# ParthaEth/GIF

Measured on AMD Instinct MI355X. Metric: G+D train-step images/sec at 256x256, batch 32/GPU, higher is better.
Workload: dtype f32

## Files before the change

### gif_amd/_lib.py

```python
import ctypes
import os

import torch

_HERE = os.path.dirname(os.path.abspath(__file__))
LIB_PATH = os.path.join(_HERE, "libgif_hip.so")

c_int, c_i64, c_float, c_void_p = ctypes.c_int, ctypes.c_int64, ctypes.c_float, ctypes.c_void_p


def knob(name, default):
    if os.environ.get("GIF_EXPERIMENTAL", "0") in ("", "0"):
        return default
    return os.environ.get(name, default)
P = c_void_p


class ConvGeom(ctypes.Structure):
    _fields_ = [(n, ctypes.c_int32) for n in ("B", "Hb", "Wb", "Cb", "Hs", "Ws", "Cs", "KH", "KW", "stride", "pad")]


class ConvEpilogue(ctypes.Structure):
    _fields_ = [("in_scale", P), ("out_scale", P), ("bias", P), ("residual", P),
                ("act", ctypes.c_int32), ("slope", c_float), ("gain", c_float),
                ("mask_src", P), ("mask_slope", c_float), ("mask_gain", c_float),
                ("dot_src", P), ("dot", P), ("colsum", P), ("red_ws", P), ("out_f32", ctypes.c_int32)]


class LinearBankSeg(ctypes.Structure):
    _fields_ = [("w", P), ("bias", P), ("s", P), ("gs", P), ("gw", P), ("gbias", P), ("n", ctypes.c_int32), ("reserved", ctypes.c_int32)]


GP, EP = ctypes.POINTER(ConvGeom), ctypes.POINTER(ConvEpilogue)

PROTOTYPES = {
    "gif_last_error": (ctypes.c_char_p, []),
    "gif_abi_version": (c_int, []),
    "gif_f16_overflow_clear": (c_int, [P]),
    "gif_f16_overflow_or_into": (c_int, [P, P]),
    "gif_f16_overflow_watch": (c_int, [c_int]),
    "gif_set_fp32_mfma_mode": (c_int, [c_int]),
    "gif_get_fp32_mfma_mode": (c_int, []),
    "gif_rasterize_workspace_bytes": (c_i64, [c_int, c_int, c_int, c_int]),
    "gif_rasterize_assume_clean_workspace": (c_int, [P, c_int]),
    "gif_rasterize_f32": (c_int, [P, P, P, P, c_int, c_int, c_int, c_int, P, P]),
    "gif_rasterize_colors_f32": (c_int, [P, P, P, P, P, c_int, c_int, c_int, c_int, P, P]),
    "gif_rasterize_f64": (c_int, [P, P, P, P, c_int, c_int, c_int, c_int, P, P]),
    "gif_rasterize_colors_f64": (c_int, [P, P, P, P, P, c_int, c_int, c_int, c_int, P, P]),
    "gif_rasterize_colors_bwd_workspace_bytes": (c_i64, [c_int, c_int, c_int, c_int]),
# ... 132 lines not shown
```

### gif_amd/csrc/common.h

```cpp
#pragma once
#include <hip/hip_runtime.h>
#include <stdint.h>
#include <stdio.h>
#include <stdlib.h>

#include "gif_hip.h"

#ifndef GIF_X3_FIRST_TERM
#define GIF_X3_FIRST_TERM 0
#endif

namespace gif {

void set_error(const char* fmt, ...);

inline int check_launch(const char* what) {
    hipError_t e = hipGetLastError();
    if (e != hipSuccess) {
        set_error("%s: %s", what, hipGetErrorString(e));
        return (int)e;
    }
    return 0;
}

#define GIF_REQUIRE(cond, ...)                \
    do {                                      \
        if (!(cond)) {                        \
            ::gif::set_error(__VA_ARGS__);    \
            return GIF_EINVAL;                \
        }                                     \
    } while (0)

inline hipStream_t as_stream(gif_stream_t s) { return reinterpret_cast<hipStream_t>(s); }

inline const char* knob(const char* name) {
    static const bool on = [] { const char* e = ::getenv("GIF_EXPERIMENTAL"); return e && atoi(e) != 0; }();
    return on ? ::getenv(name) : nullptr;
}

inline int cdiv(long a, long b) { return (int)((a + b - 1) / b); }

#if defined(__HIP_DEVICE_COMPILE__)
typedef __amdgpu_buffer_rsrc_t buf_rsrc_t;
__device__ __forceinline__ buf_rsrc_t make_buf_rsrc(const void* base, unsigned bytes) {
    return __builtin_amdgcn_make_buffer_rsrc(const_cast<void*>(base), 0, bytes, 0x00020000);
}
__device__ __forceinline__ void buf_load_lds16(buf_rsrc_t r, __attribute__((address_space(3))) void* lds, unsigned voff, int soff) {
    __builtin_amdgcn_raw_ptr_buffer_load_lds(r, lds, 16, (int)voff, soff, 0, 0);
}
#else
struct buf_rsrc_t {};
__device__ __forceinline__ buf_rsrc_t make_buf_rsrc(const void*, unsigned) { return {}; }
__device__ __forceinline__ void buf_load_lds16(buf_rsrc_t, __attribute__((address_space(3))) void*, unsigned, int) {}
#endif

constexpr int kMaxDevices = 64;
int current_device();
const float* zero_page16();
unsigned* f16_sat_flag();
struct LdsAttr {
    unsigned long granted[kMaxDevices] = {};
    void ensure(const void* kernel, size_t bytes);
};
// ... 114 lines not shown
```

### gif_amd/csrc/conv_igemm.hip

```cpp
#include <stdlib.h>

#include <atomic>
#include <type_traits>

#include "common.h"

#ifdef GIF_X3_TIMING_PROBE
__device__ unsigned long long g_x3_probe[12];
extern "C" int gif_debug_x3_probe_read(unsigned long long* out8, int reset) {
    hipDeviceSynchronize();
    if (hipMemcpyFromSymbol(out8, HIP_SYMBOL(g_x3_probe), 96) != hipSuccess) return -1;
    if (reset) {
        unsigned long long z[12] = {0, 0, 0, 0, 0, 0, 0, 0, 0, 0, 0, 0};
        if (hipMemcpyToSymbol(HIP_SYMBOL(g_x3_probe), z, 96) != hipSuccess) return -1;
    }
    return 0;
}
#endif

namespace {

typedef float f32x16 __attribute__((ext_vector_type(16)));
typedef float f32x4 __attribute__((ext_vector_type(4)));

// ... 7 lines not shown
    const float* bias;
    const void* residual;
    int B, Hi, Wi, Ci;
    int Ho, Wo, Co;
    int Hp, Wp;
    int os, ooy, oox;
    int is;
    int ntaps, nky, nkx, dy0, ddy, dx0, ddx, ky0, kx0, kstep, KW;
    int RP, CP;
    int act;
    float slope, gain;
    int M;
    int tiles_m, tiles_n;
    int stab_nb, stab_stride;
    const void* zero;
    int m_begin;
    int x3;
    const int* wexp;
    unsigned* gate;
    unsigned gate_gen;
    unsigned* h2_stats;
    const void* mask_src;
    const void* dot_src;
    float mask_slope, mask_gain;
    float* part_cs;
    float* part_dot;
    int part_row0;
    int part_cap;
    int no_split;
    unsigned* sat_flag;
    int out_f32;
    int pair;
    int dense;
    int t2_tx, t2_ty;
    int halo_dbg;
};

thread_local int t_part_rows = 0;
thread_local int t_last_bm = 0;

__device__ __forceinline__ int xcd_remap(int bid, int nwg) {
    const int nx = 8;
    int xcd = bid % nx, idx = bid / nx;
    int q = nwg / nx, r = nwg % nx;
    int base = xcd < r ? xcd * (q + 1) : r * (q + 1) + (xcd - r) * q;
    return base + idx;
// ... 6 lines not shown
    const T* const res = static_cast<const T*>(p.residual);
    T* const yout = static_cast<T*>(p.y);
    constexpr int LDC = BN + 4;
    constexpr int ROWTAB = 3;
    constexpr int STAGE_FLOATS = LDS_FLOATS ? LDS_FLOATS : 2 * (BM + BN) * LD;
    constexpr int EPI_CHUNKS = (BM * (LDC + ROWTAB) <= STAGE_FLOATS) ? 1 : (BM / 2 * (LDC + ROWTAB) <= STAGE_FLOATS) ? 2
                               : (BM / 4 * (LDC + ROWTAB) <= STAGE_FLOATS) ? 4 : 8;
    constexpr int CR = BM / EPI_CHUNKS;
    static_assert(CR % 32 == 0 && CR * (LDC + ROWTAB) <= STAGE_FLOATS && CR <= THREADS, "epilogue chunk must fit the staging LDS");
    float* Cs = smem;
    unsigned long long* const roff = reinterpret_cast<unsigned long long*>(Cs + CR * LDC);
    int* const rsmp = reinterpret_cast<int*>(roff + CR);
    constexpr unsigned long long NO_ROW = ~0ull;
    constexpr int C4_ROW = BN / 4;
    constexpr int EROWS = THREADS / C4_ROW;
    constexpr int E_IT = CR / EROWS;
    static_assert(CR % EROWS == 0, "epilogue row mapping");
    const int e_row0 = tid / C4_ROW, e_c = (tid % C4_ROW) * 4;
    const int n = n0 + e_c;
    float4 bias4 = make_float4(0.f, 0.f, 0.f, 0.f);
    if (p.bias && n < p.Co) bias4 = *reinterpret_cast<const float4*>(p.bias + n);
    const T* const msk = static_cast<const T*>(p.mask_src);
    const T* const dsrc = static_cast<const T*>(p.dot_src);
    const bool fused = msk || dsrc || p.part_cs || p.part_dot;
#if defined(GIF_EPI_PROBE) && GIF_EPI_PROBE == 3
    {
        float sacc = 0.f;
#pragma unroll
        for (int i = 0; i < MT; ++i)
#pragma unroll
            for (int j = 0; j < NT; ++j)
#pragma unroll
                for (int r = 0; r < 16; ++r) sacc += acc[i][j][r];
        if (m0 + wm0 < p.M) yout[(size_t)(m0 + wm0) * p.Co + n0 + wn0 + (tid & 63)] = (T)sacc;
        return;
    }
#endif
    float4 cs = make_float4(0.f, 0.f, 0.f, 0.f), ds = make_float4(0.f, 0.f, 0.f, 0.f);
    int osb = 0;
    f32x4 osc0 = {1.f, 1.f, 1.f, 1.f}, osc1 = osc0;
    constexpr bool OSC = sizeof(T) == 4;
    if (OSC && p.out_scale && n < p.Co) {
        osb = T2D ? t2_b : (m0 < p.M ? m0 : p.M - 1) / HWp;
        osc0 = *reinterpret_cast<const f32x4*>(p.out_scale + (size_t)osb * p.Co + n);
        osc1 = *reinterpret_cast<const f32x4*>(p.out_scale + (size_t)(osb + 1 < p.B ? osb + 1 : osb) * p.Co + n);
    }
// ... 71 lines not shown
                    for (int k = 0; k < PF; ++k) {
                        if (!ok[k]) continue;
                        float4 v = vv[k];
                        if constexpr (sizeof(T) != 4) v = *reinterpret_cast<const float4*>(Cs + (e_row0 + (it0 + k) * EROWS) * LDC + e_c);
                        if (FUSED && dsrc) {
                            ds.x += v.x * xa[k].x; ds.y += v.y * xa[k].y; ds.z += v.z * xa[k].z; ds.w += v.w * xa[k].w;
                        }
                        if (p.out_scale) {
                            f32x4 d = bs[k] == osb ? os0 : os1;
                            if (!OSC || __builtin_expect(bs[k] > osb + 1, 0)) d = *reinterpret_cast<const f32x4*>(p.out_scale + (size_t)bs[k] * p.Co + n);
                            const float dx = d[0], dy = d[1], dz = d[2], dw = d[3];
                            v.x *= dx; v.y *= dy; v.z *= dz; v.w *= dw;
                        }
                        if (res) {
                            float4 rv = gif::load4(res + off[k]);
                            v.x += rv.x; v.y += rv.y; v.z += rv.z; v.w += rv.w;
                        }
                        v.x += bias4.x; v.y += bias4.y; v.z += bias4.z; v.w += bias4.w;
                        if (p.act) {
                            v.x = (v.x > 0.f ? v.x : v.x * p.slope) * p.gain; v.y = (v.y > 0.f ? v.y : v.y * p.slope) * p.gain;
                            v.z = (v.z > 0.f ? v.z : v.z * p.slope) * p.gain; v.w = (v.w > 0.f ? v.w : v.w * p.slope) * p.gain;
                        }
                        if (FUSED) {
                            if (msk) {
                                const float4 xs = two_src ? xb[k] : xa[k];
                                v.x *= p.mask_gain * (xs.x > 0.f ? 1.f : p.mask_slope); v.y *= p.mask_gain * (xs.y > 0.f ? 1.f : p.mask_slope);
                                v.z *= p.mask_gain * (xs.z > 0.f ? 1.f : p.mask_slope); v.w *= p.mask_gain * (xs.w > 0.f ? 1.f : p.mask_slope);
                            }
                            cs.x += v.x; cs.y += v.y; cs.z += v.z; cs.w += v.w;
                        }
#ifdef GIF_NOSTORE_PROBE
                        if (p.M < 0)
#endif
                        {
                            if (sizeof(T) == 2 && p.out_f32) gif::store4(static_cast<float*>(p.y) + off[k], v);
                            else gif::store4_flag(yout + off[k], v, p.sat_flag);
                        }
                    }
                }
            };
            if (fused) rows(std::true_type{});
            else rows(std::false_type{});
        }
    }
    if (p.part_cs || p.part_dot) {
        __syncthreads();
// ... 1611 lines not shown
    GIF_REQUIRE(g->KH >= 1 && g->KH <= 3 && g->KW >= 1 && g->KW <= 3, "%s: kernel %dx%d unsupported", who, g->KH, g->KW);
    GIF_REQUIRE(g->stride == 1 || g->stride == 2, "%s: stride %d unsupported", who, g->stride);
    GIF_REQUIRE(g->pad >= 0, "%s: negative pad", who);
    GIF_REQUIRE((g->Hs - 1) * g->stride + g->KH - g->pad <= g->Hb + g->pad &&
                    (g->Ws - 1) * g->stride + g->KW - g->pad <= g->Wb + g->pad,
                "%s: small grid %dx%d does not fit big grid %dx%d (k=%d s=%d p=%d)", who, g->Hs, g->Ws, g->Hb,
                g->Wb, g->KH, g->stride, g->pad);
    return 0;
}

void fill_epilogue(GatherParams& p, const gif_conv_epilogue* e) {
    p.in_scale = e ? e->in_scale : nullptr;
    p.out_scale = e ? e->out_scale : nullptr;
    p.bias = e ? e->bias : nullptr;
    p.residual = e ? e->residual : nullptr;
    p.act = e ? e->act : 0;
    p.slope = e ? e->slope : 0.f;
    p.gain = e ? e->gain : 1.f;
    p.mask_src = e ? e->mask_src : nullptr;
    p.mask_slope = e ? e->mask_slope : 1.f;
    p.mask_gain = e ? e->mask_gain : 1.f;
    p.dot_src = e ? e->dot_src : nullptr;
    p.sat_flag = nullptr;
    p.out_f32 = e ? e->out_f32 : 0;
}

int check_tapdense(const gif_conv_geom* g, const gif_conv_epilogue* e, int cin, bool transposed, const char* who) {
    GIF_REQUIRE(gif_conv2d_x3_tapdense_steps(cin, g->KH, g->KW) > 0, "%s: tap-dense mode needs a 3x3 kernel and 8 <= Cin < 32 (got %dx%d, %d)",
                who, g->KH, g->KW, cin);
    GIF_REQUIRE(!transposed || g->stride == 1, "%s: tap-dense mode: a strided data gradient runs tap subsets per output phase", who);
    GIF_REQUIRE(!(e && e->in_scale), "%s: tap-dense mode has no per-sample input scales", who);
    return 0;
}

struct FusedSums {
    float* colsum = nullptr;
    float* dot = nullptr;
    float* part_cs = nullptr;
    float* part_dot = nullptr;
    float* tmp = nullptr;
    long cap = 0;

    bool active() const { return colsum || dot; }

    int begin(GatherParams& p, const gif_conv_epilogue* e, long out_rows, int Co, int B, long hw, bool single_phase, const char* who) {
        t_part_rows = 0;
        if (!e || (!e->colsum && !e->dot)) return 0;
// ... 48 lines not shown
        p.gate = gt.word; p.gate_gen = gt.gen;
        p.h2_stats = gif::h2_stats_words();
    }
    return 0;
}
inline void h2_to_fallback(GatherParams& p, const void* wp3) {
    p.x3 = 1;
    p.wp = wp3;
    p.wexp = nullptr;
}

template <typename T>
int check_channels(const gif_conv_geom* g, const char* who) {
    if (sizeof(T) == 2)
        GIF_REQUIRE(g->Cb % 8 == 0 && g->Cs % 8 == 0, "%s: f16 channel counts must be multiples of 8 (Cb=%d Cs=%d)", who, g->Cb, g->Cs);
    return 0;
}

template <typename T>
int conv2d_fwd_impl(const void* big, const void* wp, void* small, const gif_conv_geom* g, const gif_conv_epilogue* e,
                    gif_stream_t stream, const char* who, int x3 = 0, bool dense = false, const void* wp_fallback = nullptr) {
    if (int rc = check_geom(g, who)) return rc;
    if (int rc = check_channels<T>(g, who)) return rc;
    if (g->B == 0) return 0;
    GIF_REQUIRE(big && wp && small, "%s: null pointer", who);
    GatherParams p{};
    p.x = big; p.wp = wp; p.y = small; p.x3 = x3;
    fill_epilogue(p, e);
    if (sizeof(T) == 2) p.sat_flag = gif::f16_sat_flag();
    p.B = g->B; p.Hi = g->Hb; p.Wi = g->Wb; p.Ci = g->Cb;
    p.Ho = g->Hs; p.Wo = g->Ws; p.Co = g->Cs;
    p.Hp = g->Hs; p.Wp = g->Ws; p.os = 1; p.ooy = 0; p.oox = 0; p.is = g->stride;
    p.nky = g->KH; p.nkx = g->KW; p.ntaps = g->KH * g->KW;
    p.dy0 = -g->pad; p.ddy = 1; p.dx0 = -g->pad; p.ddx = 1;
    p.ky0 = 0; p.kx0 = 0; p.kstep = 1; p.KW = g->KW;
    pack_dims<T>(p.Co, p.Ci, &p.RP, &p.CP, x3 != 0);
    p.pair = (sizeof(T) == 2 && p.CP == 32) ? 1 : 0;
    if (dense) {
        if (int rc = check_tapdense(g, e, g->Cb, false, who)) return rc;
        p.dense = g->Cb / 4;
    }
    if (x3 == 2)
        if (int rc = h2_operands(p, wp, wp_fallback, gif::as_stream(stream))) return rc;
    p.M = p.B * p.Hp * p.Wp;
    double flops = 2.0 * p.M * (double)p.Co * p.Ci * p.ntaps;
    const int fam = sizeof(T) == 2 ? 6 : dense ? (x3 == 2 ? 17 : 12) : x3 == 2 ? 13 : x3 ? 8 : (p.Ci >= 32 ? 0 : 5);
// ... 1 lines not shown
    if (int rc = sums.begin(p, e, p.M, p.Co, p.B, (long)p.Hp * p.Wp, true, who)) return rc;
    gif::ProfScope prof(fam, flops, gif::as_stream(stream), p.M, p.Co, p.Ci, p.ntaps * 10 + g->stride);
    if (int rc = launch<T>(p, gif::as_stream(stream))) return rc;
    if (x3 == 2 && p.gate && wp_fallback) {
        const int rows2 = t_part_rows, bm2 = t_last_bm;
        h2_to_fallback(p, wp_fallback);
        t_part_rows = 0;
        if (int rc = launch<T>(p, gif::as_stream(stream))) return rc;
        if (sums.active() && (t_part_rows != rows2 || t_last_bm != bm2)) {
            gif::set_error("%s: the guarded bf16x3 twin tiles the op differently from the f16x2 launch (%d x %d vs %d x %d rows): fused "
                           "column sums would mix partials", who, t_part_rows, t_last_bm, rows2, bm2);
            return GIF_ENOSUP;
        }
    }
    if (int rc = sums.finish(p.Co, p.B, (long)p.Hp * p.Wp, gif::as_stream(stream), who)) return rc;
    return gif::check_launch(who);
}

template <typename T>
int conv2d_bwd_data_impl(const void* small, const void* wp, void* big, const gif_conv_geom* g, const gif_conv_epilogue* e,
                         gif_stream_t stream, const char* who, int x3 = 0, bool dense = false, const void* wp_fallback = nullptr) {
    if (int rc = check_geom(g, who)) return rc;
    if (int rc = check_channels<T>(g, who)) return rc;
    if (g->B == 0) return 0;
    GIF_REQUIRE(small && wp && big, "%s: null pointer", who);
    hipStream_t s = gif::as_stream(stream);
    GatherParams base{};
    base.x = small; base.wp = wp; base.y = big; base.x3 = x3;
    fill_epilogue(base, e);
    if (sizeof(T) == 2) base.sat_flag = gif::f16_sat_flag();
    base.B = g->B; base.Hi = g->Hs; base.Wi = g->Ws; base.Ci = g->Cs;
    base.Ho = g->Hb; base.Wo = g->Wb; base.Co = g->Cb;
    pack_dims<T>(base.Co, base.Ci, &base.RP, &base.CP, x3 != 0);
    base.pair = (sizeof(T) == 2 && base.CP == 32) ? 1 : 0;
    if (x3 == 2)
        if (int rc = h2_operands(base, wp, wp_fallback, s)) return rc;
    if (dense) {
        if (int rc = check_tapdense(g, e, g->Cs, true, who)) return rc;
        base.dense = g->Cs / 4;
    }
    const int st = g->stride;
    FusedSums sums;
    if (int rc = sums.begin(base, e, (long)g->B * g->Hb * g->Wb, base.Co, g->B, (long)g->Hb * g->Wb, st == 1, who)) return rc;
    auto pmod = [st](int a) { return ((a % st) + st) % st; };
    GatherParams ph[4];
    int nph = 0;
    bool need_zero = false;
    for (int py = 0; py < st; ++py)
        for (int px = 0; px < st; ++px) {
            GatherParams p = base;
            p.Hp = (g->Hb - py + st - 1) / st;
            p.Wp = (g->Wb - px + st - 1) / st;
            if (p.Hp <= 0 || p.Wp <= 0) continue;
            p.os = st; p.ooy = py; p.oox = px; p.is = 1;
            p.ky0 = pmod(py + g->pad); p.kx0 = pmod(px + g->pad); p.kstep = st; p.KW = g->KW;
            p.nky = p.ky0 < g->KH ? (g->KH - p.ky0 + st - 1) / st : 0;
            p.nkx = p.kx0 < g->KW ? (g->KW - p.kx0 + st - 1) / st : 0;
            p.ntaps = p.nky * p.nkx;
            p.dy0 = (py + g->pad - p.ky0) / st; p.ddy = -1;
            p.dx0 = (px + g->pad - p.kx0) / st; p.ddx = -1;
            if (p.ntaps == 0) { need_zero = true; continue; }
            p.M = p.B * p.Hp * p.Wp;
            ph[nph++] = p;
        }
    if (need_zero) {
        GIF_REQUIRE(!(e && (e->bias || e->residual || e->act || e->mask_src || e->colsum || e->dot)), "%s: epilogue unsupported with empty phases", who);
        hipError_t me = hipMemsetAsync(big, 0, (size_t)g->B * g->Hb * g->Wb * g->Cb * sizeof(T), s);
        if (me != hipSuccess) { gif::set_error("%s memset: %s", who, hipGetErrorString(me)); return (int)me; }
    }
    double flops = 2.0 * g->B * (double)g->Hs * g->Ws * g->KH * g->KW * (double)g->Cs * g->Cb;
    {
        const int fam = sizeof(T) == 2 ? 6 : dense ? (x3 == 2 ? 17 : 12) : x3 == 2 ? 13 : x3 ? 8 : (base.Ci >= 32 ? 0 : 5);
        gif::ProfScope prof(fam, flops, s, g->B * g->Hb * g->Wb, base.Co, base.Ci, -(g->KH * g->KW * 10 + g->stride));
        auto run_phases = [&]() -> int {
            bool merged = false;
            if (nph > 1 && conv_variant() == 0) {
                TileCfg c = pick_cfg<T>(base.Co, base.Ci);
                if (x3) c.BK = 32;
                bool small_all = c.BN == 128 && (sizeof(T) == 2 || c.BK == 32);
                for (int i = 0; i < nph && small_all; ++i)
                    small_all = (long)gif::cdiv(ph[i].M, 128) * (ph[i].RP / 128) < 384 &&
                                (long)ph[i].B * ph[i].Hi * ph[i].Wi * ph[i].Ci < (1L << 31) &&
                                (long)ph[i].B * ph[i].Ho * ph[i].Wo * ph[i].Co < (1L << 31);
                if (small_all)
                    merged = launch_multi<T>(ph, nph, base.in_scale != nullptr, s) == 0;
                if constexpr (sizeof(T) == 4) {
                    static const int big_multi_off = gif::knob("GIF_X3_MULTI_BIG") ? atoi(gif::knob("GIF_X3_MULTI_BIG")) == 0 : 0;
                    bool big_all = x3 && !small_all && !big_multi_off && c.BN == 128;
                    for (int i = 0; i < nph && big_all; ++i)
// ... 135 lines not shown
```

### gif_amd/csrc/conv_winograd.hip

```cpp
#include <stdlib.h>
#include <string.h>

#include "common.h"

namespace {

typedef float f32x16 __attribute__((ext_vector_type(16)));
typedef float f32x4 __attribute__((ext_vector_type(4)));

__device__ __forceinline__ int xcd_remap(int bid, int nwg) {
    const int nx = 8;
    int xcd = bid % nx, idx = bid / nx;
    int q = nwg / nx, r = nwg % nx;
    int base = xcd < r ? xcd * (q + 1) : r * (q + 1) + (xcd - r) * q;
    return base + idx;
}

constexpr int WBM = 128, WBN = 64, WBK = 32, WNSTAGE = 3;
constexpr int WPAD = 256;

__global__ void __launch_bounds__(256) wino_input_transform(const float* __restrict__ x, const float* __restrict__ scale,
                                                            float* __restrict__ V, int B, int H, int W, int C, int CP,
                                                            long ntiles_pad) {
    const int C4 = CP >> 2, TH = H >> 1, TW = W >> 1;
// ... 174 lines not shown
        U[(i * 4 + 1) * plane + idx] = 0.5f * (u[i][0] + u[i][1] + u[i][2]);
        U[(i * 4 + 2) * plane + idx] = 0.5f * (u[i][0] - u[i][1] + u[i][2]);
        U[(i * 4 + 3) * plane + idx] = u[i][2];
    }
}

struct WinoParams {
    const float* V;
    const float* U;
    float* y;
    const float* out_scale;
    const float* bias;
    const float* residual;
    int B, H, W, Co, RP, CP;
    int ntiles, ntiles_pad, TH, TW;
    int act;
    float slope, gain;
    int tiles_m, tiles_n;
    const float* mask_src;
    const float* dot_src;
    float mask_slope, mask_gain;
    float* part_cs;
    float* part_dot;
    const int* uexp;
    unsigned* gate;
    unsigned gate_gen;
    unsigned* h2_stats;
};

template <bool FUSED, int E_IT, int EROWS, int LDC, int PF>
__device__ __forceinline__ void wino_epilogue_rows(const WinoParams& p, const float* Cs, int m0, int e_row0, int e_c, int n, int oa, int ob,
                                                   const f32x4& bias4, f32x4& cs, f32x4& ds, const unsigned long long* rtab = nullptr,
                                                   const int* rsmp = nullptr) {
    static_assert(E_IT % PF == 0, "epilogue batches");
    const bool two_src = FUSED && p.mask_src && p.dot_src && p.mask_src != p.dot_src;
    const size_t pos_off = ((size_t)oa * p.W + ob) * p.Co + n;
#pragma unroll 1
    for (int it0 = 0; it0 < E_IT; it0 += PF) {
        size_t off[PF];
        bool ok[PF];
        f32x4 rv[PF], dv[PF], xa[PF], xb[PF];
#pragma unroll
        for (int k = 0; k < PF; ++k) {
            int b;
            if (rtab) {
                const int row = e_row0 + (it0 + k) * EROWS;
// ... 12 lines not shown
            }
            rv[k] = dv[k] = xa[k] = xb[k] = (f32x4)(0.f);
            if (ok[k]) {
                if (p.residual) rv[k] = *reinterpret_cast<const f32x4*>(p.residual + off[k]);
                if (p.out_scale) dv[k] = *reinterpret_cast<const f32x4*>(p.out_scale + (size_t)b * p.Co + n);
                if (FUSED && p.dot_src) xa[k] = *reinterpret_cast<const f32x4*>(p.dot_src + off[k]);
                if (FUSED && p.mask_src && !p.dot_src) xa[k] = *reinterpret_cast<const f32x4*>(p.mask_src + off[k]);
                if (two_src) xb[k] = *reinterpret_cast<const f32x4*>(p.mask_src + off[k]);
            }
        }
#pragma unroll
        for (int k = 0; k < PF; ++k) {
            if (!ok[k]) continue;
            f32x4 v = *reinterpret_cast<const f32x4*>(Cs + (e_row0 + (it0 + k) * EROWS) * LDC + e_c);
            if (FUSED && p.dot_src) ds += v * xa[k];
            if (p.out_scale) v *= dv[k];
            if (p.residual) v += rv[k];
            v += bias4;
            if (p.act) {
#pragma unroll
                for (int e = 0; e < 4; ++e) v[e] = (v[e] > 0.f ? v[e] : v[e] * p.slope) * p.gain;
            }
            if (FUSED) {
                if (p.mask_src) {
                    const f32x4 xs = two_src ? xb[k] : xa[k];
#pragma unroll
                    for (int e = 0; e < 4; ++e) v[e] *= p.mask_gain * (xs[e] > 0.f ? 1.f : p.mask_slope);
                }
                cs += v;
            }
            *reinterpret_cast<f32x4*>(p.y + off[k]) = v;
        }
    }
}

template <int THREADS, int C4_ROW, int EROWS>
__device__ __forceinline__ void wino_write_partials(const WinoParams& p, float* smem, int tid, int n, int prow, f32x4 cs, f32x4 ds) {
    if (!p.part_cs && !p.part_dot) return;
    __syncthreads();
    f32x4* red = reinterpret_cast<f32x4*>(smem);
    red[tid] = cs;
    red[THREADS + tid] = ds;
    __syncthreads();
    if (tid < C4_ROW && n < p.Co) {
        f32x4 a = red[tid], b = red[THREADS + tid];
#pragma unroll
// ... 867 lines not shown
    return 16 * ntiles_pad * CP;
}

int gif_winograd_weight_f32(const float* w, float* U, int R, int C, int RP, int CP, int64_t sr, int64_t sc, int64_t sky,
                            int64_t skx, int flip, float scale, gif_stream_t stream) {
    GIF_REQUIRE(w && U && R > 0 && C > 0 && RP >= R && CP >= C, "winograd_weight: bad arguments");
    long total = (long)RP * CP;
    wino_weight_transform<<<gif::cdiv(total, 256), 256, 0, gif::as_stream(stream)>>>(w, U, R, C, RP, CP, sr, sc, sky, skx,
                                                                                      flip, scale);
    return gif::check_launch("winograd_weight");
}

}

namespace {

struct WinoSums {
    float *colsum = nullptr, *dot = nullptr, *tmp = nullptr;
    int begin(WinoParams& p, const gif_conv_epilogue* e, int B, int H, int W, int Co, int bm, const char* who) {
        p.mask_src = e ? static_cast<const float*>(e->mask_src) : nullptr;
        p.mask_slope = e ? e->mask_slope : 1.f;
        p.mask_gain = e ? e->mask_gain : 1.f;
        p.dot_src = e ? static_cast<const float*>(e->dot_src) : nullptr;
        if (!e || (!e->colsum && !e->dot)) return 0;
        GIF_REQUIRE(e->red_ws, "%s: colsum / dot need the red_ws workspace (gif_conv_epilogue_ws_floats)", who);
        const long per_sample = (long)(H / 2) * (W / 2);
        GIF_REQUIRE(!e->dot || (e->dot_src && per_sample % bm == 0),
                    "%s: the dot fusion needs dot_src and a multiple of %d 2x2 tiles per sample (got %ld)", who, bm, per_sample);
        const long cap = (long)B * H * W / 64 + 16;
        GIF_REQUIRE(p.tiles_m <= cap, "%s: partial-sum rows exceed the workspace", who);
        colsum = e->colsum;
        dot = e->dot;
        p.part_cs = colsum ? e->red_ws : nullptr;
        p.part_dot = dot ? e->red_ws + cap * Co : nullptr;
        tmp = e->red_ws + 2 * cap * Co;
        return 0;
    }
    int finish(const WinoParams& p, int B, int H, int W, int Co, int bm, hipStream_t s) {
        if (colsum)
            if (int rc = gif::reduce_partials(p.part_cs, colsum, 1, p.tiles_m, Co, tmp, s)) return rc;
        if (dot) {
            const int per = (int)((long)(H / 2) * (W / 2) / bm);
            if (int rc = gif::reduce_partials(p.part_dot, dot, B, per, Co, tmp, s)) return rc;
        }
        return 0;
    }
// ... 185 lines not shown
```

### gif_amd/csrc/elementwise.hip

```cpp
#include "common.h"

namespace {

__device__ __forceinline__ float wave_sum(float v) {
#pragma unroll
    for (int off = 32; off > 0; off >>= 1) v += __shfl_xor(v, off, 64);
    return v;
}

__device__ __forceinline__ float4 f4add(float4 a, float4 b) { return make_float4(a.x + b.x, a.y + b.y, a.z + b.z, a.w + b.w); }
__device__ __forceinline__ float4 f4fma(float s, float4 a, float4 c) {
    return make_float4(fmaf(s, a.x, c.x), fmaf(s, a.y, c.y), fmaf(s, a.z, c.z), fmaf(s, a.w, c.w));
}
__device__ __forceinline__ float lrelu(float v, float slope, float gain) { return (v > 0.f ? v : v * slope) * gain; }

template <typename T>
struct UpfirdnParams {
    const T* x;
    const float* k;
    T* y;
    const float* bias;
    const T* residual;
    int B, Hi, Wi, C, Ho, Wo, up, down, padx0, pady0, KH, KW, flip, act;
    float slope, gain;
// ... 603 lines not shown
            int ry = iy % f - o0, rx = ix % f - o0;
            if ((ry == 0 || ry == 1) && (rx == 0 || rx == 1)) {
                float4 g = reinterpret_cast<const float4*>(gy)[(((size_t)b * S + iy / f) * S + ix / f) * C4 + c4];
                r = make_float4(0.25f * g.x, 0.25f * g.y, 0.25f * g.z, 0.25f * g.w);
            }
        }
        reinterpret_cast<float4*>(gx)[idx] = r;
    }
}

inline int ew_grid(long n) {
    long b = (n + 255) / 256;
    if (b > 256 * 16) b = 256 * 16;
    if (b < 1) b = 1;
    return (int)b;
}

template <typename T>
int upfirdn2d_impl(const T* x, const float* k, T* y, int B, int Hi, int Wi, int C, int Ho, int Wo, int up, int down, int padx0,
                   int pady0, int KH, int KW, int flip, const gif_conv_epilogue* e, gif_stream_t stream) {
    GIF_REQUIRE(x && k && y, "upfirdn2d: null pointer");
    GIF_REQUIRE(B >= 0 && Hi > 0 && Wi > 0 && Ho > 0 && Wo > 0 && C > 0 && C % 4 == 0, "upfirdn2d: bad dims (C=%d)", C);
    GIF_REQUIRE(up >= 1 && down >= 1 && KH >= 1 && KW >= 1 && KH * KW <= 16, "upfirdn2d: bad up/down/kernel");
    if (B == 0) return 0;
    UpfirdnParams<T> p{};
    p.x = x; p.k = k; p.y = y;
    p.bias = e ? e->bias : nullptr;
    p.residual = e ? static_cast<const T*>(e->residual) : nullptr;
    p.act = e ? e->act : 0;
    p.slope = e ? e->slope : 0.f;
    p.gain = e ? e->gain : 1.f;
    p.B = B; p.Hi = Hi; p.Wi = Wi; p.C = C; p.Ho = Ho; p.Wo = Wo; p.up = up; p.down = down;
    p.padx0 = padx0; p.pady0 = pady0; p.KH = KH; p.KW = KW; p.flip = flip;
    p.sat_flag = sizeof(T) == 2 ? gif::f16_sat_flag() : nullptr;
    const bool blur = up == 1 && down == 1 && KH == 4 && KW == 4;
    const bool fused = e && (e->mask_src || e->colsum || e->dot || e->dot_src);
    float* colsum_out = nullptr;
    if (fused) {
        GIF_REQUIRE(!e->dot && !e->dot_src, "upfirdn2d: the dot fusion is a convolution epilogue only");
        GIF_REQUIRE(blur, "upfirdn2d: mask / colsum fusions need the 4x4 blur form (up = down = 1)");
        GIF_REQUIRE(!e->colsum || (e->red_ws && (C & (C - 1)) == 0 && C <= 1024), "upfirdn2d: colsum needs red_ws and a power-of-two C <= 1024");
        p.mask_src = static_cast<const T*>(e->mask_src);
        p.mask_slope = e->mask_slope; p.mask_gain = e->mask_gain;
        colsum_out = e->colsum;
        p.part_cs = colsum_out ? e->red_ws : nullptr;
    }
// ... 429 lines not shown
```

### gif_amd/functional.py

```python
import torch
from torch.autograd import Function

from . import ops
from .ops import ConvSpec


class ActPort:
    __slots__ = ("alias", "slope", "gain", "want_bias", "parts")

    def __init__(self, slope, gain, want_bias):
        self.alias, self.slope, self.gain, self.want_bias = None, float(slope), float(gain), bool(want_bias)
        self.parts = []

    def cfg(self):
        return (self.slope, self.gain, self.want_bias, self.parts)


def _take_port(x, identity=False):
    port = getattr(x, "_gif_port", None)
    if (port is None or not ops.FUSE_GRAD or not torch.is_grad_enabled() or port.alias is None or not port.alias.requires_grad
            or (port.slope == 1.0 and port.gain == 1.0) != identity):
        return None, None
    return port.alias, port.cfg()


_inputs_only = False


class inputs_only_backward:
    def __enter__(self):
        global _inputs_only
        self._prev, _inputs_only = _inputs_only, True

    def __exit__(self, *exc):
        global _inputs_only
        _inputs_only = self._prev


# ... 40 lines not shown
        parts.append(gb)
    return gxm


def _producer_gpre(gy, g_port, y, want_b, slope, gain, parts):
    gpre = gb = None
    if gy is not None:
        gpre, gb = BiasActBwdFn.apply(gy, y, want_b, slope, gain)
        if not want_b:
            gb = None
    if g_port is not None:
        gpre = g_port if gpre is None else gpre + g_port
        if want_b and parts:
            for part in parts:
                gb = part if gb is None else gb + part
    if parts is not None:
        parts.clear()
    return gpre, gb


class Conv2dFn(Function):

    @staticmethod
    def forward(ctx, x, w, spec, transposed, out_hw, wscale, residual=None):
        ctx.pmask = _param_mask(x, w)
        x = ops.nhwc(x)
        ctx.spec, ctx.transposed, ctx.wscale = spec, transposed, wscale
        ctx.save_for_backward(x, w)
        ctx.v = None
        epi = {} if residual is None else {"residual": ops.nhwc(residual)}
        if not transposed:
            y, v = ops.conv_fwd(x, w, spec, wscale, keep_v=True, **epi)
            ctx.v = v if ctx.needs_input_grad[1] else None
            return y
        return ops.conv_bwd_data(x, w, spec, tuple(out_hw), wscale, **epi)

    @staticmethod
    def backward(ctx, gy):
        x, w = ctx.saved_tensors
        spec, tr, ws = ctx.spec, ctx.transposed, ctx.wscale
        gx = gw = gr = None
        if _need(ctx, 0):
            gx = Conv2dFn.apply(gy, w, spec, not tr, tuple(x.shape[2:]), ws, None)
            assert gx.shape == x.shape, (gx.shape, x.shape)
        if _need(ctx, 1):
            O, I = w.shape[:2]
            gw = WgradFn.apply(gy, x, spec, O, I, ws, ctx.v) if not tr else WgradFn.apply(x, gy, spec, O, I, ws)
        if ctx.needs_input_grad[6]:
            gr = gy
        return gx, gw, None, None, None, None, gr


class WgradFn(Function):

    @staticmethod
    def forward(ctx, small, big, spec, O, I, wscale, big_v=None):
        small, big = ops.nhwc(small), ops.nhwc(big)
        ctx.spec, ctx.wscale = spec, wscale
        ctx.save_for_backward(small, big)
        return ops.conv_wgrad(small, big, spec, O, I, wscale, big_v=big_v)

    @staticmethod
    def backward(ctx, ggw):
        small, big = ctx.saved_tensors
        gs = gb = None
        if ctx.needs_input_grad[0]:
            gs = Conv2dFn.apply(big, ggw, ctx.spec, False, None, ctx.wscale, None)
        if ctx.needs_input_grad[1]:
            gb = Conv2dFn.apply(small, ggw, ctx.spec, True, tuple(big.shape[2:]), ctx.wscale, None)
        return gs, gb, None, None, None, None, None


class ConvBiasActFn(Function):

    @staticmethod
    def forward(ctx, x, w, bias, spec, wscale, slope, gain, passthrough=False, in_port=None, parts=None, x_port=None):
        ctx.set_materialize_grads(False)
        ctx.pmask = _param_mask(x, w, bias)
        x = ops.nhwc(x)
        y, v = ops.conv_fwd(x, w, spec, wscale, keep_v=True, bias=bias, act=True, slope=slope, gain=gain)
        ctx.v = v if ctx.needs_input_grad[1] else None
        ctx.cfg = (spec, wscale, slope, gain, bias is not None)
        ctx.in_port, ctx.parts = in_port, parts
        ctx.save_for_backward(x, w, y)
        return y, y.detach(), (x.view_as(x) if passthrough else None)

    @staticmethod
    def backward(ctx, gy, g_port=None, g_alias=None):
        x, w, y = ctx.saved_tensors
        spec, ws, slope, gain, has_bias = ctx.cfg
        want_b = has_bias and _need(ctx, 2)
        gx = gw = None
        port = _port_on(ctx)
        gpre, gb = _producer_gpre(gy, g_port, y, want_b, slope, gain, ctx.parts)
        if gpre is not None:
            if ctx.needs_input_grad[0]:
                gx = _conv_dgrad(gpre, w, spec, tuple(x.shape[2:]), ws, g_alias, ctx.in_port if port else None, x)
            if _need(ctx, 1):
                gw = WgradFn.apply(gpre, x, spec, w.shape[0], w.shape[1], ws, ctx.v)
        elif ctx.needs_input_grad[0] and g_alias is not None:
            gx = _mask_into_port(ctx.in_port, g_alias, x) if port else g_alias
        return (None if port else gx), gw, (gb if want_b else None), None, None, None, None, None, None, None, (gx if port else None)


def _conv_dgrad(gpre, w, spec, big_hw, ws, residual, in_port, x):
    if in_port is None:
        return Conv2dFn.apply(gpre, w, spec, True, big_hw, ws, residual)
    slope, gain, want_b, parts = in_port
    fuse = ops.GradFuse(mask_src=x, mask_slope=slope, mask_gain=gain, want_colsum=want_b)
    gx = ops.conv_bwd_data(gpre, w, spec, big_hw, ws, residual=None if residual is None else ops.nhwc(residual), fuse=fuse)
    if want_b:
        parts.append(fuse.colsum)
    return gx


def conv2d_bias_act(x, w, bias, stride=1, pad=0, wscale=1.0, slope=0.2, gain=2 ** 0.5, passthrough=False):
    x_port, in_port = _take_port(x)
    port = _new_port(True, slope, gain, bias)
    y, alias, x_alias = ConvBiasActFn.apply(x, w, bias, ConvSpec(w.shape[2], w.shape[3], stride, pad), wscale, slope, gain,
                                            bool(passthrough), in_port, None if port is None else port.parts, x_port)
    _tag(y, alias, port)
    return (y, x_alias) if passthrough else y


def conv2d(x, w, stride=1, pad=0, wscale=1.0, residual=None):
    return Conv2dFn.apply(x, w, ConvSpec(w.shape[2], w.shape[3], stride, pad), False, None, wscale, residual)


def conv_transpose2d(x, w, stride, pad, out_hw, wscale=1.0):
    return Conv2dFn.apply(x, w, ConvSpec(w.shape[2], w.shape[3], stride, pad), True, tuple(out_hw), wscale, None)


class LinearNtFn(Function):

    @staticmethod
    def forward(ctx, a, b, scale, n_pad):
        ctx.scale = scale
        ctx.pmask = _param_mask(a, b)
        ctx.save_for_backward(a, b)
        return ops.linear_nt(a, b, None, scale, n_pad=n_pad)

    @staticmethod
    def backward(ctx, g):
        a, b = ctx.saved_tensors
        N, K = b.shape
        ga = LinearNnFn.apply(g, b, ctx.scale, a.shape[1]) if _need(ctx, 0) else None
        gb = LinearTnFn.apply(g, a, ctx.scale, N, K) if _need(ctx, 1) else None
        return ga, gb, None, None

# ... 580 lines not shown
```

### gif_amd/ops.py

```python
import ctypes
import functools
import os
import weakref
from typing import NamedTuple, Optional

import torch

from . import _lib

CL = torch.channels_last


def _stream():
    return torch.cuda.current_stream().cuda_stream


def _device_guard(fn):
    @functools.wraps(fn)
    def wrapped(*args, **kw):
        dev = None
        for a in args + tuple(kw.values()):
            if isinstance(a, torch.Tensor) and a.is_cuda:
                if dev is None:
                    dev = a.device
# ... 48 lines not shown
    return torch.empty((B, C, H, W), device=device, dtype=dtype, memory_format=CL)


class ConvSpec(NamedTuple):
    KH: int
    KW: int
    stride: int
    pad: int

    def small_hw(self, Hb, Wb):
        return ((Hb + 2 * self.pad - self.KH) // self.stride + 1, (Wb + 2 * self.pad - self.KW) // self.stride + 1)

    def big_hw(self, Hs, Ws):
        return ((Hs - 1) * self.stride + self.KH - 2 * self.pad, (Ws - 1) * self.stride + self.KW - 2 * self.pad)


def _geom(B, Hb, Wb, Cb, Hs, Ws, Cs, spec: ConvSpec):
    return _lib.ConvGeom(B, Hb, Wb, Cb, Hs, Ws, Cs, spec.KH, spec.KW, spec.stride, spec.pad)


FUSE_GRAD = _lib.knob("GIF_FUSE_GRAD", "1") != "0"


class GradFuse:

    def __init__(self, mask_src=None, mask_slope=1.0, mask_gain=1.0, want_colsum=False, dot_src=None):
        self.mask_src, self.mask_slope, self.mask_gain = mask_src, float(mask_slope), float(mask_gain)
        self.want_colsum, self.dot_src = bool(want_colsum), dot_src
        self.colsum = self.dot = self._ws = None


def dot_fusable(H, W, dtype=torch.float32):
    return FUSE_GRAD and dtype in (torch.float32, torch.float16) and (H * W) % 1024 == 0


def _epilogue(in_scale=None, out_scale=None, bias=None, residual=None, act=False, slope=0.2, gain=2 ** 0.5, fuse=None,
              out_bchw=None, dtype=torch.float32, out_f32=False):
    e = _lib.ConvEpilogue(_p(in_scale), _p(out_scale), _p(bias), _p(residual), 1 if act else 0, slope, gain)
    e.out_f32 = 1 if out_f32 else 0
    if fuse is not None:
        B, C, H, W = out_bchw
        for t, what in ((fuse.mask_src, "mask_src"), (fuse.dot_src, "dot_src")):
            if t is not None and (tuple(t.shape) != (B, C, H, W) or t.dtype != dtype or not t.is_contiguous(memory_format=CL)):
                raise _lib.GifHipError(f"GradFuse.{what}: expected an NHWC {dtype} tensor of shape {(B, C, H, W)}, got {tuple(t.shape)} {t.dtype}")
        e.mask_src, e.mask_slope, e.mask_gain = _p(fuse.mask_src), fuse.mask_slope, fuse.mask_gain
        e.dot_src = _p(fuse.dot_src)
        if fuse.mask_src is None and fuse.dot_src is None:
            raise _lib.GifHipError("GradFuse: nothing to fuse (the plain column sum of a gradient is ops.colsum)")
        device = fuse.mask_src.device if fuse.mask_src is not None else fuse.dot_src.device
        if fuse.dot_src is not None:
            fuse.dot = torch.empty((B, C), device=device, dtype=torch.float32)
            e.dot = fuse.dot.data_ptr()
        if fuse.want_colsum:
            fuse.colsum = torch.empty((C,), device=device, dtype=torch.float32)
            e.colsum = fuse.colsum.data_ptr()
        if fuse.dot is not None or fuse.colsum is not None:
            fuse._ws = torch.empty((_lib.load().gif_conv_epilogue_ws_floats(B * H * W, C),), device=device, dtype=torch.float32)
            e.red_ws = fuse._ws.data_ptr()
    return e


WEIGHT_CACHE = _lib.knob("GIF_WEIGHT_CACHE", "1") != "0"
_weight_cache = {}
_WEIGHT_CACHE_MAX = 512


def clear_weight_cache():
    _weight_cache.clear()


def _cached_weight_op(w, tag, build):
    if not WEIGHT_CACHE:
        return build()
    base = w._base if w._base is not None else w
    key = (id(base), tag, w.storage_offset(), tuple(w.shape), tuple(w.stride()))
    state = (base.data_ptr(), base._version)
    hit = _weight_cache.get(key)
    if hit is not None and hit[0]() is base and hit[1] == state:
# ... 821 lines not shown
```

### include/gif_hip.h

```cpp
#ifndef GIF_HIP_H
#define GIF_HIP_H

#include <stdint.h>

#ifdef __cplusplus
extern "C" {
#endif

#define GIF_EINVAL (-1)
#define GIF_ENOSUP (-2)

typedef void* gif_stream_t;

const char* gif_last_error(void);
int gif_abi_version(void);

int gif_f16_overflow_clear(gif_stream_t stream);
int gif_f16_overflow_or_into(float* found_inf, gif_stream_t stream);
int gif_f16_overflow_watch(int on);

#define GIF_FP32_MFMA_NATIVE 0
#define GIF_FP32_MFMA_BF16X3 1
#define GIF_FP32_MFMA_F16X2 2
int gif_set_fp32_mfma_mode(int mode);
// ... 52 lines not shown
typedef struct {
    int32_t B;
    int32_t Hb, Wb, Cb;
    int32_t Hs, Ws, Cs;
    int32_t KH, KW;
    int32_t stride;
    int32_t pad;
} gif_conv_geom;

typedef struct {
    const float* in_scale;
    const float* out_scale;
    const float* bias;
    const void* residual;
    int32_t act;
    float slope, gain;
    const void* mask_src;
    float mask_slope, mask_gain;
    const void* dot_src;
    float* dot;
    float* colsum;
    float* red_ws;
    int32_t out_f32;
} gif_conv_epilogue;
int64_t gif_conv_epilogue_ws_floats(int64_t out_rows, int cout);

int gif_conv2d_pack_dims(int cout, int cin, int* RP, int* CP);
int gif_pack_weight_f32(const float* w, float* wp, int R, int C, int KH, int KW, int RP, int CP, int64_t sr,
                        int64_t sc, int64_t sky, int64_t skx, float scale, gif_stream_t stream);
int gif_conv2d_fwd_f32(const float* big, const float* wp, float* small, const gif_conv_geom* g,
                       const gif_conv_epilogue* e, gif_stream_t stream);
int gif_conv2d_bwd_data_f32(const float* small, const float* wp, float* big, const gif_conv_geom* g,
                            const gif_conv_epilogue* e, gif_stream_t stream);
int gif_conv2d_fwd_f32x3(const float* big, const void* wp3, float* small, const gif_conv_geom* g, const gif_conv_epilogue* e,
                         gif_stream_t stream);
int gif_conv2d_bwd_data_f32x3(const float* small, const void* wp3, float* big, const gif_conv_geom* g,
                              const gif_conv_epilogue* e, gif_stream_t stream);
int gif_conv2d_fwd_f32h2(const float* big, const void* wp2, const void* wp3, float* small, const gif_conv_geom* g,
                         const gif_conv_epilogue* e, gif_stream_t stream);
int gif_conv2d_bwd_data_f32h2(const float* small, const void* wp2, const void* wp3, float* big, const gif_conv_geom* g,
                              const gif_conv_epilogue* e, gif_stream_t stream);
int gif_conv2d_fwd_f32h2_tapdense(const float* big, const void* wp2, const void* wp3, float* small, const gif_conv_geom* g,
                                  const gif_conv_epilogue* e, gif_stream_t stream);
int gif_conv2d_bwd_data_f32h2_tapdense(const float* small, const void* wp2, const void* wp3, float* big, const gif_conv_geom* g,
                                       const gif_conv_epilogue* e, gif_stream_t stream);
int gif_conv2d_fwd_f32x3_tapdense(const float* big, const void* wp3, float* small, const gif_conv_geom* g,
                                  const gif_conv_epilogue* e, gif_stream_t stream);
// ... 165 lines not shown
```

Measured before the change: 179.0.

## Add dual-output conv dgrad epilogue to relay residual and masked gradients

Adds an out_plain output to the conv epilogue so a single backward-data convolution writes both the plain gradient and the leaky-ReLU-masked gradient. The autograd path gets a relay mechanism: when a conv with residual follows a bias-act conv, the next bias-act conv's dgrad emits both gradients at once. This removes a separate dgrad or elementwise pass over the gradient tensor on that path. In exchange it writes an extra full-size tensor, extends the ABI struct, and adds autograd plumbing complexity.

```diff
diff --git a/gif_amd/_lib.py b/gif_amd/_lib.py
--- a/gif_amd/_lib.py
+++ b/gif_amd/_lib.py
@@ -24,7 +24,10 @@
     _fields_ = [("in_scale", P), ("out_scale", P), ("bias", P), ("residual", P),
                 ("act", ctypes.c_int32), ("slope", c_float), ("gain", c_float),
                 ("mask_src", P), ("mask_slope", c_float), ("mask_gain", c_float),
-                ("dot_src", P), ("dot", P), ("colsum", P), ("red_ws", P), ("out_f32", ctypes.c_int32)]
+                ("dot_src", P), ("dot", P), ("colsum", P), ("red_ws", P), ("out_f32", ctypes.c_int32), ("out_plain", P)]
+
+
+EPI_OUT_F32, EPI_REV5 = 1, 2
 
 
 class LinearBankSeg(ctypes.Structure):
diff --git a/gif_amd/csrc/common.h b/gif_amd/csrc/common.h
--- a/gif_amd/csrc/common.h
+++ b/gif_amd/csrc/common.h
@@ -39,6 +39,8 @@
 }
 
 inline int cdiv(long a, long b) { return (int)((a + b - 1) / b); }
+
+inline void* epi_out_plain(const gif_conv_epilogue* e) { return (e && (e->out_f32 & GIF_EPI_REV5)) ? e->out_plain : nullptr; }
 
 #if defined(__HIP_DEVICE_COMPILE__)
 typedef __amdgpu_buffer_rsrc_t buf_rsrc_t;
diff --git a/gif_amd/csrc/conv_igemm.hip b/gif_amd/csrc/conv_igemm.hip
--- a/gif_amd/csrc/conv_igemm.hip
+++ b/gif_amd/csrc/conv_igemm.hip
@@ -53,6 +53,7 @@
     unsigned* h2_stats;
     const void* mask_src;
     const void* dot_src;
+    void* y_plain;
     float mask_slope, mask_gain;
     float* part_cs;
     float* part_dot;
@@ -105,6 +106,7 @@
     if (p.bias && n < p.Co) bias4 = *reinterpret_cast<const float4*>(p.bias + n);
     const T* const msk = static_cast<const T*>(p.mask_src);
     const T* const dsrc = static_cast<const T*>(p.dot_src);
+    T* const yplain = static_cast<T*>(p.y_plain);
     const bool fused = msk || dsrc || p.part_cs || p.part_dot;
 #if defined(GIF_EPI_PROBE) && GIF_EPI_PROBE == 3
     {
@@ -222,6 +224,7 @@
                             v.z = (v.z > 0.f ? v.z : v.z * p.slope) * p.gain; v.w = (v.w > 0.f ? v.w : v.w * p.slope) * p.gain;
                         }
                         if (FUSED) {
+                            if (yplain) gif::store4_flag(yplain + off[k], v, p.sat_flag);
                             if (msk) {
                                 const float4 xs = two_src ? xb[k] : xa[k];
                                 v.x *= p.mask_gain * (xs.x > 0.f ? 1.f : p.mask_slope); v.y *= p.mask_gain * (xs.y > 0.f ? 1.f : p.mask_slope);
@@ -1879,7 +1882,16 @@
     p.mask_gain = e ? e->mask_gain : 1.f;
     p.dot_src = e ? e->dot_src : nullptr;
     p.sat_flag = nullptr;
-    p.out_f32 = e ? e->out_f32 : 0;
+    p.out_f32 = e ? (e->out_f32 & GIF_EPI_OUT_F32) : 0;
+    p.y_plain = gif::epi_out_plain(e);
+}
+
+template <typename T>
+int check_out_plain(const gif_conv_epilogue* e, const char* who) {
+    if (!gif::epi_out_plain(e)) return 0;
+    if (sizeof(T) != 4) { gif::set_error("%s: out_plain is not supported by the f16 kernels", who); return GIF_ENOSUP; }
+    GIF_REQUIRE(e->mask_src, "%s: out_plain needs mask_src (without a mask both outputs would be the same tensor)", who);
+    return 0;
 }
 
 int check_tapdense(const gif_conv_geom* g, const gif_conv_epilogue* e, int cin, bool transposed, const char* who) {
@@ -1974,6 +1986,7 @@
                     gif_stream_t stream, const char* who, int x3 = 0, bool dense = false, const void* wp_fallback = nullptr) {
     if (int rc = check_geom(g, who)) return rc;
     if (int rc = check_channels<T>(g, who)) return rc;
+    if (int rc = check_out_plain<T>(e, who)) return rc;
     if (g->B == 0) return 0;
     GIF_REQUIRE(big && wp && small, "%s: null pointer", who);
     GatherParams p{};
@@ -2021,6 +2034,7 @@
                          gif_stream_t stream, const char* who, int x3 = 0, bool dense = false, const void* wp_fallback = nullptr) {
     if (int rc = check_geom(g, who)) return rc;
     if (int rc = check_channels<T>(g, who)) return rc;
+    if (int rc = check_out_plain<T>(e, who)) return rc;
     if (g->B == 0) return 0;
     GIF_REQUIRE(small && wp && big, "%s: null pointer", who);
     hipStream_t s = gif::as_stream(stream);
@@ -2063,7 +2077,7 @@
             ph[nph++] = p;
         }
     if (need_zero) {
-        GIF_REQUIRE(!(e && (e->bias || e->residual || e->act || e->mask_src || e->colsum || e->dot)), "%s: epilogue unsupported with empty phases", who);
+        GIF_REQUIRE(!(e && (e->bias || e->residual || e->act || e->mask_src || e->colsum || e->dot || gif::epi_out_plain(e))), "%s: epilogue unsupported with empty phases", who);
         hipError_t me = hipMemsetAsync(big, 0, (size_t)g->B * g->Hb * g->Wb * g->Cb * sizeof(T), s);
         if (me != hipSuccess) { gif::set_error("%s memset: %s", who, hipGetErrorString(me)); return (int)me; }
     }
diff --git a/gif_amd/csrc/conv_winograd.hip b/gif_amd/csrc/conv_winograd.hip
--- a/gif_amd/csrc/conv_winograd.hip
+++ b/gif_amd/csrc/conv_winograd.hip
@@ -220,6 +220,7 @@
     float mask_slope, mask_gain;
     float* part_cs;
     float* part_dot;
+    float* y_plain;
     const int* uexp;
     unsigned* gate;
     unsigned gate_gen;
@@ -278,6 +279,7 @@
                 for (int e = 0; e < 4; ++e) v[e] = (v[e] > 0.f ? v[e] : v[e] * p.slope) * p.gain;
             }
             if (FUSED) {
+                if (p.y_plain) *reinterpret_cast<f32x4*>(p.y_plain + off[k]) = v;
                 if (p.mask_src) {
                     const f32x4 xs = two_src ? xb[k] : xa[k];
 #pragma unroll
@@ -1191,6 +1193,8 @@
         p.mask_slope = e ? e->mask_slope : 1.f;
         p.mask_gain = e ? e->mask_gain : 1.f;
         p.dot_src = e ? static_cast<const float*>(e->dot_src) : nullptr;
+        p.y_plain = static_cast<float*>(gif::epi_out_plain(e));
+        GIF_REQUIRE(!p.y_plain || p.mask_src, "%s: out_plain needs mask_src (without a mask both outputs would be the same tensor)", who);
         if (!e || (!e->colsum && !e->dot)) return 0;
         GIF_REQUIRE(e->red_ws, "%s: colsum / dot need the red_ws workspace (gif_conv_epilogue_ws_floats)", who);
         const long per_sample = (long)(H / 2) * (W / 2);
diff --git a/gif_amd/csrc/elementwise.hip b/gif_amd/csrc/elementwise.hip
--- a/gif_amd/csrc/elementwise.hip
+++ b/gif_amd/csrc/elementwise.hip
@@ -649,6 +649,7 @@
     GIF_REQUIRE(x && k && y, "upfirdn2d: null pointer");
     GIF_REQUIRE(B >= 0 && Hi > 0 && Wi > 0 && Ho > 0 && Wo > 0 && C > 0 && C % 4 == 0, "upfirdn2d: bad dims (C=%d)", C);
     GIF_REQUIRE(up >= 1 && down >= 1 && KH >= 1 && KW >= 1 && KH * KW <= 16, "upfirdn2d: bad up/down/kernel");
+    if (gif::epi_out_plain(e)) { gif::set_error("upfirdn2d: out_plain (epilogue revision 5) is a convolution epilogue only"); return GIF_ENOSUP; }
     if (B == 0) return 0;
     UpfirdnParams<T> p{};
     p.x = x; p.k = k; p.y = y;
diff --git a/gif_amd/functional.py b/gif_amd/functional.py
--- a/gif_amd/functional.py
+++ b/gif_amd/functional.py
@@ -14,6 +14,21 @@
 
     def cfg(self):
         return (self.slope, self.gain, self.want_bias, self.parts)
+
+
+class RelayPort:
+    __slots__ = ("alias", "mask_alias", "mask_src", "cfg")
+
+    def __init__(self, alias, mask_alias, mask_src, cfg):
+        self.alias, self.mask_alias, self.mask_src, self.cfg = alias, mask_alias, mask_src, cfg
+
+
+def _take_relay(x):
+    relay = getattr(x, "_gif_relay", None)
+    if (relay is None or not torch.is_grad_enabled() or not ops.dual_fusable(x) or not relay.alias.requires_grad
+            or not relay.mask_alias.requires_grad):
+        return None
+    return relay
 
 
 def _take_port(x, identity=False):
@@ -100,7 +115,11 @@
 class Conv2dFn(Function):
 
     @staticmethod
-    def forward(ctx, x, w, spec, transposed, out_hw, wscale, residual=None):
+    def forward(ctx, x, w, spec, transposed, out_hw, wscale, residual=None, relay=False):
+        ctx.relay = bool(relay)
+        if relay:
+            assert not transposed
+            ctx.set_materialize_grads(False)
         ctx.pmask = _param_mask(x, w)
         x = ops.nhwc(x)
         ctx.spec, ctx.transposed, ctx.wscale = spec, transposed, wscale
@@ -110,14 +129,20 @@
         if not transposed:
             y, v = ops.conv_fwd(x, w, spec, wscale, keep_v=True, **epi)
             ctx.v = v if ctx.needs_input_grad[1] else None
-            return y
+            return (y, y.detach()) if relay else y
         return ops.conv_bwd_data(x, w, spec, tuple(out_hw), wscale, **epi)
 
     @staticmethod
-    def backward(ctx, gy):
+    def backward(ctx, gy, g_relay=None):
         x, w = ctx.saved_tensors
         spec, tr, ws = ctx.spec, ctx.transposed, ctx.wscale
         gx = gw = gr = None
+        if ctx.relay:
+            g_res, gy = gy, (g_relay if gy is None else gy if g_relay is None else gy + g_relay)
+            if gy is None:
+                return (None,) * 8
+        else:
+            g_res = gy
         if _need(ctx, 0):
             gx = Conv2dFn.apply(gy, w, spec, not tr, tuple(x.shape[2:]), ws, None)
             assert gx.shape == x.shape, (gx.shape, x.shape)
@@ -125,8 +150,8 @@
             O, I = w.shape[:2]
             gw = WgradFn.apply(gy, x, spec, O, I, ws, ctx.v) if not tr else WgradFn.apply(x, gy, spec, O, I, ws)
         if ctx.needs_input_grad[6]:
-            gr = gy
-        return gx, gw, None, None, None, None, gr
+            gr = g_res
+        return gx, gw, None, None, None, None, gr, None
 
 
 class WgradFn(Function):
@@ -152,33 +177,52 @@
 class ConvBiasActFn(Function):
 
     @staticmethod
-    def forward(ctx, x, w, bias, spec, wscale, slope, gain, passthrough=False, in_port=None, parts=None, x_port=None):
+    def forward(ctx, x, w, bias, spec, wscale, slope, gain, passthrough=False, in_port=None, parts=None, x_port=None,
+                relay=None, x_relay=None, m_alias=None, m_src=None):
+        assert relay is None or in_port is None
         ctx.set_materialize_grads(False)
         ctx.pmask = _param_mask(x, w, bias)
         x = ops.nhwc(x)
         y, v = ops.conv_fwd(x, w, spec, wscale, keep_v=True, bias=bias, act=True, slope=slope, gain=gain)
         ctx.v = v if ctx.needs_input_grad[1] else None
         ctx.cfg = (spec, wscale, slope, gain, bias is not None)
-        ctx.in_port, ctx.parts = in_port, parts
-        ctx.save_for_backward(x, w, y)
+        ctx.in_port, ctx.parts, ctx.relay = in_port, parts, relay
+        ctx.save_for_backward(x, w, y, *(() if relay is None else (m_src,)))
         return y, y.detach(), (x.view_as(x) if passthrough else None)
 
     @staticmethod
     def backward(ctx, gy, g_port=None, g_alias=None):
-        x, w, y = ctx.saved_tensors
+        x, w, y = ctx.saved_tensors[:3]
         spec, ws, slope, gain, has_bias = ctx.cfg
         want_b = has_bias and _need(ctx, 2)
-        gx = gw = None
+        gx = gw = gxm = None
         port = _port_on(ctx)
+        relay = ctx.relay is not None and not torch.is_grad_enabled()
         gpre, gb = _producer_gpre(gy, g_port, y, want_b, slope, gain, ctx.parts)
         if gpre is not None:
-            if ctx.needs_input_grad[0]:
+            if ctx.needs_input_grad[0] and relay:
+                gx, gxm = _conv_dgrad_dual(gpre, w, spec, tuple(x.shape[2:]), ws, g_alias, ctx.relay, ctx.saved_tensors[3])
+            elif ctx.needs_input_grad[0]:
                 gx = _conv_dgrad(gpre, w, spec, tuple(x.shape[2:]), ws, g_alias, ctx.in_port if port else None, x)
             if _need(ctx, 1):
                 gw = WgradFn.apply(gpre, x, spec, w.shape[0], w.shape[1], ws, ctx.v)
         elif ctx.needs_input_grad[0] and g_alias is not None:
             gx = _mask_into_port(ctx.in_port, g_alias, x) if port else g_alias
-        return (None if port else gx), gw, (gb if want_b else None), None, None, None, None, None, None, None, (gx if port else None)
+        if gxm is not None:
+            return None, gw, (gb if want_b else None), None, None, None, None, None, None, None, None, None, gx, gxm, None
+        return ((None if port else gx), gw, (gb if want_b else None), None, None, None, None, None, None, None, (gx if port else None),
+                None, None, None, None)
+
+
+def _conv_dgrad_dual(gpre, w, spec, big_hw, ws, residual, relay_cfg, m_src):
+    slope, gain, want_b, parts = relay_cfg
+    fuse = ops.GradFuse(mask_src=m_src, mask_slope=slope, mask_gain=gain, want_colsum=want_b, want_plain=True)
+    gxm = ops.conv_bwd_data(gpre, w, spec, big_hw, ws, residual=None if residual is None else ops.nhwc(residual), fuse=fuse)
+    if fuse.plain is None:
+        raise RuntimeError("conv_bwd_data did not produce the plain output of a dual-output epilogue")
+    if want_b:
+        parts.append(fuse.colsum)
+    return fuse.plain, gxm
 
 
 def _conv_dgrad(gpre, w, spec, big_hw, ws, residual, in_port, x):
@@ -194,15 +238,24 @@
 
 def conv2d_bias_act(x, w, bias, stride=1, pad=0, wscale=1.0, slope=0.2, gain=2 ** 0.5, passthrough=False):
     x_port, in_port = _take_port(x)
+    relay = _take_relay(x) if in_port is None else None
     port = _new_port(True, slope, gain, bias)
+    rl = (None, None, None, None) if relay is None else (relay.cfg, relay.alias, relay.mask_alias, relay.mask_src)
     y, alias, x_alias = ConvBiasActFn.apply(x, w, bias, ConvSpec(w.shape[2], w.shape[3], stride, pad), wscale, slope, gain,
-                                            bool(passthrough), in_port, None if port is None else port.parts, x_port)
+                                            bool(passthrough), in_port, None if port is None else port.parts, x_port, *rl)
     _tag(y, alias, port)
     return (y, x_alias) if passthrough else y
 
 
 def conv2d(x, w, stride=1, pad=0, wscale=1.0, residual=None):
-    return Conv2dFn.apply(x, w, ConvSpec(w.shape[2], w.shape[3], stride, pad), False, None, wscale, residual)
+    spec = ConvSpec(w.shape[2], w.shape[3], stride, pad)
+    if residual is not None and ops.dual_fusable(residual):
+        r_alias, r_cfg = _take_port(residual)
+        if r_alias is not None:
+            z, z_alias = Conv2dFn.apply(x, w, spec, False, None, wscale, residual, True)
+            z._gif_relay = RelayPort(z_alias, r_alias, residual.detach(), r_cfg)
+            return z
+    return Conv2dFn.apply(x, w, spec, False, None, wscale, residual)
 
 
 def conv_transpose2d(x, w, stride, pad, out_hw, wscale=1.0):
diff --git a/gif_amd/ops.py b/gif_amd/ops.py
--- a/gif_amd/ops.py
+++ b/gif_amd/ops.py
@@ -94,12 +94,20 @@
 FUSE_GRAD = _lib.knob("GIF_FUSE_GRAD", "1") != "0"
 
 
+DUAL_EPILOGUE = _lib.knob("GIF_DUAL_EPILOGUE", "1") != "0"
+DUAL_STATS = {"launches": 0}
+
+
+def dual_fusable(x):
+    return FUSE_GRAD and DUAL_EPILOGUE and x.is_cuda and x.dtype == torch.float32
+
+
 class GradFuse:
 
-    def __init__(self, mask_src=None, mask_slope=1.0, mask_gain=1.0, want_colsum=False, dot_src=None):
+    def __init__(self, mask_src=None, mask_slope=1.0, mask_gain=1.0, want_colsum=False, dot_src=None, want_plain=False):
         self.mask_src, self.mask_slope, self.mask_gain = mask_src, float(mask_slope), float(mask_gain)
-        self.want_colsum, self.dot_src = bool(want_colsum), dot_src
-        self.colsum = self.dot = self._ws = None
+        self.want_colsum, self.dot_src, self.want_plain = bool(want_colsum), dot_src, bool(want_plain)
+        self.colsum = self.dot = self.plain = self._ws = None
 
 
 def dot_fusable(H, W, dtype=torch.float32):
@@ -109,7 +117,7 @@
 def _epilogue(in_scale=None, out_scale=None, bias=None, residual=None, act=False, slope=0.2, gain=2 ** 0.5, fuse=None,
               out_bchw=None, dtype=torch.float32, out_f32=False):
     e = _lib.ConvEpilogue(_p(in_scale), _p(out_scale), _p(bias), _p(residual), 1 if act else 0, slope, gain)
-    e.out_f32 = 1 if out_f32 else 0
+    e.out_f32 = _lib.EPI_OUT_F32 if out_f32 else 0
     if fuse is not None:
         B, C, H, W = out_bchw
         for t, what in ((fuse.mask_src, "mask_src"), (fuse.dot_src, "dot_src")):
@@ -126,6 +134,13 @@
         if fuse.want_colsum:
             fuse.colsum = torch.empty((C,), device=device, dtype=torch.float32)
             e.colsum = fuse.colsum.data_ptr()
+        if fuse.want_plain:
+            if fuse.mask_src is None or dtype != torch.float32:
+                raise _lib.GifHipError("GradFuse.want_plain needs mask_src and fp32 tensors")
+            fuse.plain = empty_nhwc(B, C, H, W, device, dtype)
+            e.out_plain = fuse.plain.data_ptr()
+            e.out_f32 |= _lib.EPI_REV5
+            DUAL_STATS["launches"] += 1
         if fuse.dot is not None or fuse.colsum is not None:
             fuse._ws = torch.empty((_lib.load().gif_conv_epilogue_ws_floats(B * H * W, C),), device=device, dtype=torch.float32)
             e.red_ws = fuse._ws.data_ptr()
diff --git a/include/gif_hip.h b/include/gif_hip.h
--- a/include/gif_hip.h
+++ b/include/gif_hip.h
@@ -98,7 +98,10 @@
     float* colsum;
     float* red_ws;
     int32_t out_f32;
+    void* out_plain;
 } gif_conv_epilogue;
+#define GIF_EPI_OUT_F32 1
+#define GIF_EPI_REV5 2
 int64_t gif_conv_epilogue_ws_floats(int64_t out_rows, int cout);
 
 int gif_conv2d_pack_dims(int cout, int cin, int* RP, int* CP);
```

Measured after the change: 178.6. Within noise of the previous version (-0.2%).
